# MDFahimAnjum/AliasFree-Diffusion-Models-PyTorch

Hardware: AMD Instinct MI355X
Metric: train_step_images_per_sec (higher is better)
Workload: dtype f32; 1 GPU; CIFAR-10 32x32x3 synthetic, UNet variant=3 (Config D), batch 256/GPU, T=1000, AdamW lr 3e-4, random-init weights (seed 42); global_batch=256, parallelism=dp1, hip_graph=True, launch_mode=lanes

## Files before the change

### aliasfree-diffusion-models-pytorch_amd/csrc/attn.hip

```cpp
#include "common.h"

namespace afd {

constexpr int kTile = 64;
constexpr int kChunk = 8;

using f2 = __attribute__((ext_vector_type(2))) float;
constexpr float kLog2e = 1.4426950408889634f, kLn2 = 0.6931471805599453f;

template <int D> struct RowVec {
  static __device__ __forceinline__ void load(const float* __restrict__ p, f2 (&v)[D / 2]) {
    if constexpr (D % 4 == 0) {
#pragma unroll
      for (int j = 0; j < D / 4; ++j) {
        const float4 t = reinterpret_cast<const float4*>(p)[j];
        v[2 * j] = (f2){t.x, t.y}; v[2 * j + 1] = (f2){t.z, t.w};
      }
    } else {
      const float2 t = *reinterpret_cast<const float2*>(p);
      v[0] = (f2){t.x, t.y};
    }
  }
};
template <int P> __device__ __forceinline__ float dot2(const f2 (&a)[P], const f2 (&b)[P]) {
  f2 t = a[0] * b[0];
#pragma unroll
  for (int i = 1; i < P; ++i) t = __builtin_elementwise_fma(a[i], b[i], t);
  return t.x + t.y;
}
template <int P> __device__ __forceinline__ void axpy2(f2 (&acc)[P], float s, const f2 (&v)[P]) {
  const f2 ss = {s, s};
#pragma unroll
  for (int i = 0; i < P; ++i) acc[i] = __builtin_elementwise_fma(ss, v[i], acc[i]);
}

template <int D, int NT>
__device__ __forceinline__ void stage_rows(const float* __restrict__ src, float* __restrict__ dst, int r0, int L, float mul) {
  constexpr int Q4 = D * kTile / 4;
  if constexpr (Q4 % NT == 0) {
    if ((L & 3) == 0) {
      constexpr int CAP = D >= 64 ? 2 : 8;
      constexpr int N4 = Q4 / NT, CH = N4 < CAP ? N4 : CAP;
#pragma unroll
      for (int e0 = 0; e0 < N4; e0 += CH) {
        float4 v[CH];
#pragma unroll
        for (int e = 0; e < CH; ++e) {
          const int i = threadIdx.x + NT * (e0 + e), j = i / (kTile / 4), rr = 4 * (i % (kTile / 4));
          v[e] = (r0 + rr < L) ? *reinterpret_cast<const float4*>(src + (long)j * L + r0 + rr) : make_float4(0.f, 0.f, 0.f, 0.f);
        }
#pragma unroll
        for (int e = 0; e < CH; ++e) {
          const int i = threadIdx.x + NT * (e0 + e), j = i / (kTile / 4), rr = 4 * (i % (kTile / 4));
          dst[rr * D + j] = v[e].x * mul; dst[(rr + 1) * D + j] = v[e].y * mul;
          dst[(rr + 2) * D + j] = v[e].z * mul; dst[(rr + 3) * D + j] = v[e].w * mul;
        }
      }
      return;
    }
  }
#pragma unroll 4
  for (int i = threadIdx.x; i < D * kTile; i += NT) {
    const int j = i / kTile, rr = i % kTile;
    dst[rr * D + j] = (r0 + rr < L) ? src[(long)j * L + r0 + rr] * mul : 0.f;
  }
}

template <int D, int R, int NT>
__global__ __launch_bounds__(NT) void attn_fwd_k(const float* __restrict__ qkv, float* __restrict__ o,
                                                  float* __restrict__ lse, int heads, int L, float scale) {
  constexpr int P = D / 2;
  __shared__ __attribute__((aligned(16))) float Ks[kTile * D];
  __shared__ __attribute__((aligned(16))) float Vs[kTile * D];
  const int b = blockIdx.z, h = blockIdx.y;
  const int C = heads * D;
  const int q0 = blockIdx.x * NT * R + threadIdx.x;
  const float* qp = qkv + ((long)b * 3 * C + h * D) * L;
  const float* kp = qp + (long)C * L;
  const float* vp = kp + (long)C * L;
  f2 q[R][P], acc[R][P];
  float m[R], l[R];
#pragma unroll
  for (int r = 0; r < R; ++r) {
    const int qi = q0 + r * NT;
    m[r] = -INFINITY; l[r] = 0.f;
#pragma unroll
    for (int j = 0; j < D; ++j) q[r][j >> 1][j & 1] = qi < L ? qp[(long)j * L + qi] * (scale * kLog2e) : 0.f;
#pragma unroll
    for (int i = 0; i < P; ++i) acc[r][i] = (f2){0.f, 0.f};
  }
  for (int k0 = 0; k0 < L; k0 += kTile) {
    __syncthreads();
    stage_rows<D, NT>(kp, Ks, k0, L, 1.f);
    stage_rows<D, NT>(vp, Vs, k0, L, 1.f);
    __syncthreads();
    const int nk = min(kTile, L - k0);
    for (int c0 = 0; c0 < nk; c0 += kChunk) {
      float s[R][kChunk], cm[R];
#pragma unroll
      for (int r = 0; r < R; ++r) cm[r] = m[r];
#pragma unroll
      for (int u = 0; u < kChunk; ++u) {
        f2 kv[P];
        RowVec<D>::load(Ks + (c0 + u) * D, kv);
        const bool in = c0 + u < nk;
#pragma unroll
        for (int r = 0; r < R; ++r) {
          s[r][u] = in ? dot2<P>(q[r], kv) : -INFINITY;
          cm[r] = fmaxf(cm[r], s[r][u]);
        }
      }
#pragma unroll
      for (int r = 0; r < R; ++r) {
        const float alpha = __builtin_amdgcn_exp2f(m[r] - cm[r]);
        l[r] *= alpha;
#pragma unroll
        for (int i = 0; i < P; ++i) acc[r][i] *= alpha;
        m[r] = cm[r];
      }
#pragma unroll
      for (int u = 0; u < kChunk; ++u) {
        f2 vv[P];
        RowVec<D>::load(Vs + (c0 + u) * D, vv);
#pragma unroll
        for (int r = 0; r < R; ++r) {
          const float p = __builtin_amdgcn_exp2f(s[r][u] - cm[r]);
          l[r] += p;
          axpy2<P>(acc[r], p, vv);
        }
      }
    }
  }
#pragma unroll
  for (int r = 0; r < R; ++r) {
    const int qi = q0 + r * NT;
    if (qi < L) {
      const float inv = 1.0f / l[r];
      float* op = o + ((long)b * C + h * D) * L + qi;
#pragma unroll
      for (int j = 0; j < D; ++j) op[(long)j * L] = acc[r][j >> 1][j & 1] * inv;
      lse[((long)b * heads + h) * L + qi] = (m[r] + __builtin_amdgcn_logf(l[r])) * kLn2;
    }
  }
}

template <int D, int R, int NT>
__global__ __launch_bounds__(NT) void attn_bwd_dq_k(const float* __restrict__ qkv, const float* __restrict__ o,
                                                     const float* __restrict__ d_o, const float* __restrict__ lse,
                                                     float* __restrict__ dqkv, float* __restrict__ delta_out,
                                                     int heads, int L, float scale) {
  constexpr int P = D / 2;
  __shared__ __attribute__((aligned(16))) float Ks[kTile * D];
  __shared__ __attribute__((aligned(16))) float Vs[kTile * D];
  const int b = blockIdx.z, h = blockIdx.y;
  const int C = heads * D;
  const int q0 = blockIdx.x * NT * R + threadIdx.x;
  const float* qp = qkv + ((long)b * 3 * C + h * D) * L;
  const float* kp = qp + (long)C * L;
  const float* vp = kp + (long)C * L;
  const long obase = ((long)b * C + h * D) * L;
  f2 q[R][P], go[R][P], dq[R][P];
  float delta[R], ls[R];
#pragma unroll
  for (int r = 0; r < R; ++r) {
    const int qi = q0 + r * NT;
    const bool live = qi < L;
    delta[r] = 0.f;
#pragma unroll
    for (int j = 0; j < D; ++j) {
      const float g = live ? d_o[obase + (long)j * L + qi] : 0.f;
      q[r][j >> 1][j & 1] = live ? qp[(long)j * L + qi] * (scale * kLog2e) : 0.f;
      go[r][j >> 1][j & 1] = g;
      delta[r] += g * (live ? o[obase + (long)j * L + qi] : 0.f);
    }
#pragma unroll
    for (int i = 0; i < P; ++i) dq[r][i] = (f2){0.f, 0.f};
    ls[r] = live ? lse[((long)b * heads + h) * L + qi] * kLog2e : 0.f;
    if (live) delta_out[((long)b * heads + h) * L + qi] = delta[r];
  }
  for (int k0 = 0; k0 < L; k0 += kTile) {
    __syncthreads();
    stage_rows<D, NT>(kp, Ks, k0, L, 1.f);
    stage_rows<D, NT>(vp, Vs, k0, L, 1.f);
    __syncthreads();
    const int nk = min(kTile, L - k0);
#pragma unroll 2
    for (int u = 0; u < nk; ++u) {
      f2 kv[P], vv[P];
      RowVec<D>::load(Ks + u * D, kv);
      RowVec<D>::load(Vs + u * D, vv);
#pragma unroll
      for (int r = 0; r < R; ++r) {
        const float sc = dot2<P>(q[r], kv), dp = dot2<P>(go[r], vv);
        const float ds = __builtin_amdgcn_exp2f(sc - ls[r]) * (dp - delta[r]);
        axpy2<P>(dq[r], ds, kv);
      }
    }
  }
#pragma unroll
  for (int r = 0; r < R; ++r) {
    const int qi = q0 + r * NT;
    if (qi < L) {
      float* dqp = dqkv + ((long)b * 3 * C + h * D) * L + qi;
#pragma unroll
      for (int j = 0; j < D; ++j) dqp[(long)j * L] = dq[r][j >> 1][j & 1] * scale;
    }
  }
}

template <int D, int R, int NT>
__global__ __launch_bounds__(NT) void attn_bwd_dkv_k(const float* __restrict__ qkv, const float* __restrict__ d_o,
                                                      const float* __restrict__ lse, const float* __restrict__ delta,
                                                      float* __restrict__ dqkv, int heads, int L, float scale) {
  constexpr int P = D / 2;
  __shared__ __attribute__((aligned(16))) float Qs[kTile * D];
  __shared__ __attribute__((aligned(16))) float Gs[kTile * D];
  __shared__ float Ls[kTile];
  __shared__ float Ds[kTile];
  const int b = blockIdx.z, h = blockIdx.y;
  const int C = heads * D;
  const int kq0 = blockIdx.x * NT * R + threadIdx.x;
  const float* qp = qkv + ((long)b * 3 * C + h * D) * L;
  const float* kp = qp + (long)C * L;
  const float* vp = kp + (long)C * L;
  const float* gp = d_o + ((long)b * C + h * D) * L;
  const float* lp = lse + ((long)b * heads + h) * L;
  const float* dlp = delta + ((long)b * heads + h) * L;
  f2 k[R][P], v[R][P], dk[R][P], dv[R][P];
#pragma unroll
  for (int r = 0; r < R; ++r) {
    const int ki = kq0 + r * NT;
#pragma unroll
    for (int j = 0; j < D; ++j) {
      k[r][j >> 1][j & 1] = ki < L ? kp[(long)j * L + ki] : 0.f;
      v[r][j >> 1][j & 1] = ki < L ? vp[(long)j * L + ki] : 0.f;
    }
#pragma unroll
    for (int i = 0; i < P; ++i) { dk[r][i] = (f2){0.f, 0.f}; dv[r][i] = (f2){0.f, 0.f}; }
  }
  for (int t0 = 0; t0 < L; t0 += kTile) {
    __syncthreads();
    stage_rows<D, NT>(qp, Qs, t0, L, scale * kLog2e);
    stage_rows<D, NT>(gp, Gs, t0, L, 1.f);
    for (int i = threadIdx.x; i < kTile; i += NT) {
      const bool in = t0 + i < L;
      Ls[i] = in ? lp[t0 + i] * kLog2e : INFINITY;
      Ds[i] = in ? dlp[t0 + i] : 0.f;
    }
    __syncthreads();
    const int nq = min(kTile, L - t0);
#pragma unroll 2
    for (int u = 0; u < nq; ++u) {
      f2 qv[P], gv[P];
      RowVec<D>::load(Qs + u * D, qv);
      RowVec<D>::load(Gs + u * D, gv);
      const float lsu = Ls[u], dlu = Ds[u];
#pragma unroll
      for (int r = 0; r < R; ++r) {
        const float sc = dot2<P>(qv, k[r]), dp = dot2<P>(gv, v[r]);
        const float p = __builtin_amdgcn_exp2f(sc - lsu);
        const float ds = p * (dp - dlu);
        axpy2<P>(dv[r], p, gv);
        axpy2<P>(dk[r], ds, qv);
      }
    }
  }
#pragma unroll
  for (int r = 0; r < R; ++r) {
    const int ki = kq0 + r * NT;
    if (ki < L) {
      float* dkp = dqkv + ((long)b * 3 * C + C + h * D) * L + ki;
      float* dvp = dkp + (long)C * L;
#pragma unroll
      for (int j = 0; j < D; ++j) { dkp[(long)j * L] = dk[r][j >> 1][j & 1] * kLn2; dvp[(long)j * L] = dv[r][j >> 1][j & 1]; }
    }
  }
}

}
using namespace afd;

template <int R> static inline void attn_geometry(int B, int heads, int L, dim3& grid, dim3& block) {
  const int rows = (L + R - 1) / R;
  block = dim3(rows <= 64 ? 64 : (rows <= 128 ? 128 : 256));
  grid = dim3((L + block.x * R - 1) / (block.x * R), heads, B);
}
template <int D, int R> static void launch_fwd(const float* qkv, float* o, float* lse, int B, int heads, int L, float sc, hipStream_t s) {
  dim3 grid, block; attn_geometry<R>(B, heads, L, grid, block);
  if (block.x == 64) hipLaunchKernelGGL((attn_fwd_k<D, R, 64>), grid, block, 0, s, qkv, o, lse, heads, L, sc);
  else if (block.x == 128) hipLaunchKernelGGL((attn_fwd_k<D, R, 128>), grid, block, 0, s, qkv, o, lse, heads, L, sc);
  else hipLaunchKernelGGL((attn_fwd_k<D, R, 256>), grid, block, 0, s, qkv, o, lse, heads, L, sc);
}
template <int D, int R> static void launch_dq(const float* qkv, const float* o, const float* d_o, const float* lse, float* dqkv,
                                              float* delta, int B, int heads, int L, float sc, hipStream_t s) {
  dim3 grid, block; attn_geometry<R>(B, heads, L, grid, block);
  if (block.x == 64) hipLaunchKernelGGL((attn_bwd_dq_k<D, R, 64>), grid, block, 0, s, qkv, o, d_o, lse, dqkv, delta, heads, L, sc);
  else if (block.x == 128) hipLaunchKernelGGL((attn_bwd_dq_k<D, R, 128>), grid, block, 0, s, qkv, o, d_o, lse, dqkv, delta, heads, L, sc);
  else hipLaunchKernelGGL((attn_bwd_dq_k<D, R, 256>), grid, block, 0, s, qkv, o, d_o, lse, dqkv, delta, heads, L, sc);
}
template <int D, int R> static void launch_dkv(const float* qkv, const float* d_o, const float* lse, const float* delta, float* dqkv,
                                               int B, int heads, int L, float sc, hipStream_t s) {
  dim3 grid, block; attn_geometry<R>(B, heads, L, grid, block);
  if (block.x == 64) hipLaunchKernelGGL((attn_bwd_dkv_k<D, R, 64>), grid, block, 0, s, qkv, d_o, lse, delta, dqkv, heads, L, sc);
  else if (block.x == 128) hipLaunchKernelGGL((attn_bwd_dkv_k<D, R, 128>), grid, block, 0, s, qkv, d_o, lse, delta, dqkv, heads, L, sc);
  else hipLaunchKernelGGL((attn_bwd_dkv_k<D, R, 256>), grid, block, 0, s, qkv, d_o, lse, delta, dqkv, heads, L, sc);
}

namespace afd {
bool attn_mfma8_ok(int d, int L);
void attn_pv_set(int m);
bool attn_fused_bwd(const float* qkv, const float* o, const float* d_o, const float* lse, float* dqkv, float* delta, int B, int heads,
                    int d, int L, float sc, hipStream_t s);
void attn_mfma8_fwd(const float* qkv, float* o, float* lse, int B, int heads, int d, int L, float sc, hipStream_t s);
void attn_mfma8_bwd_dq(const float* qkv, const float* o, const float* d_o, const float* lse, float* dqkv, float* delta,
                       int B, int heads, int d, int L, float sc, hipStream_t s);
void attn_mfma8_bwd_dkv(const float* qkv, const float* d_o, const float* lse, const float* delta, float* dqkv, int B, int heads, int L,
                        float sc, hipStream_t s);
}
static int g_attn_mfma_bwd_all = 1;
static int g_attn_rows = 0;

extern "C" {

int afd_debug_attn_rows(int r) {
  if (r == 20 || r == 21) { attn_pv_set(r - 20); return AFD_OK; }
  if (r == 10 || r == 11) { g_attn_mfma_bwd_all = r - 10; return AFD_OK; }
  AFD_REQUIRE(r == 0 || r == 1 || r == 2 || r == 4, "afd_debug_attn_rows: r must be 0, 1, 2, 4 (rows per lane of the VALU kernels), 10, 11, 20 or 21");
  g_attn_rows = r;
  return AFD_OK;
}

int afd_attn_fwd(const float* qkv, float* o, float* lse, int B, int heads, int d, int L, afd_stream_t st) {
  AFD_REQUIRE(qkv && o && lse && B > 0 && heads > 0 && L > 0, "afd_attn_fwd: bad argument");
  AFD_REQUIRE(d == 2 || d == 4 || d == 8 || d == 16 || d == 32 || d == 64, "afd_attn_fwd: head dim %d not in {2,4,8,16,32,64}", d);
  AFD_REQUIRE(B <= 65535 && heads <= 65535, "afd_attn_fwd: grid too large");
  hipStream_t s = as_stream(st);
  const float sc = 1.0f / sqrtf((float)d);
  if (g_attn_rows == 0 && attn_mfma8_ok(d, L)) { attn_mfma8_fwd(qkv, o, lse, B, heads, d, L, sc, s); return check_launch("afd_attn_fwd"); }
  switch (d) {
    case 2:  launch_fwd<2, 4>(qkv, o, lse, B, heads, L, sc, s); break;
    case 4:  launch_fwd<4, 4>(qkv, o, lse, B, heads, L, sc, s); break;
    case 8:
      if (g_attn_rows == 1 || (g_attn_rows == 0 && L < 1024)) launch_fwd<8, 1>(qkv, o, lse, B, heads, L, sc, s);
      else if (g_attn_rows == 4) launch_fwd<8, 4>(qkv, o, lse, B, heads, L, sc, s);
      else launch_fwd<8, 2>(qkv, o, lse, B, heads, L, sc, s);
      break;
    case 16: if (L <= 64) launch_fwd<16, 1>(qkv, o, lse, B, heads, L, sc, s); else launch_fwd<16, 2>(qkv, o, lse, B, heads, L, sc, s); break;
    case 32: if (L <= 64) launch_fwd<32, 1>(qkv, o, lse, B, heads, L, sc, s); else launch_fwd<32, 2>(qkv, o, lse, B, heads, L, sc, s); break;
    default: launch_fwd<64, 1>(qkv, o, lse, B, heads, L, sc, s); break;
  }
  return check_launch("afd_attn_fwd");
}

int afd_attn_bwd(const float* qkv, const float* o, const float* d_o, const float* lse, float* dqkv, float* delta_ws,
                 int B, int heads, int d, int L, afd_stream_t st) {
  AFD_REQUIRE(qkv && o && d_o && lse && dqkv && delta_ws && B > 0 && heads > 0 && L > 0, "afd_attn_bwd: bad argument");
  AFD_REQUIRE(d == 2 || d == 4 || d == 8 || d == 16 || d == 32 || d == 64, "afd_attn_bwd: head dim %d not in {2,4,8,16,32,64}", d);
  AFD_REQUIRE(B <= 65535 && heads <= 65535, "afd_attn_bwd: grid too large");
  hipStream_t s = as_stream(st);
  const float sc = 1.0f / sqrtf((float)d);
  if (g_attn_rows == 0 && attn_mfma8_ok(d, L) && (L < 1024 || g_attn_mfma_bwd_all)) {
    if (attn_fused_bwd(qkv, o, d_o, lse, dqkv, delta_ws, B, heads, d, L, sc, s)) return check_launch("afd_attn_bwd");
    attn_mfma8_bwd_dq(qkv, o, d_o, lse, dqkv, delta_ws, B, heads, d, L, sc, s);
    if (d == 8) attn_mfma8_bwd_dkv(qkv, d_o, lse, delta_ws, dqkv, B, heads, L, sc, s);
    else launch_dkv<16, 2>(qkv, d_o, lse, delta_ws, dqkv, B, heads, L, sc, s);
    return check_launch("afd_attn_bwd");
  }
  switch (d) {
    case 2:  launch_dq<2, 4>(qkv, o, d_o, lse, dqkv, delta_ws, B, heads, L, sc, s); break;
    case 4:  launch_dq<4, 4>(qkv, o, d_o, lse, dqkv, delta_ws, B, heads, L, sc, s); break;
    case 8:
      if (g_attn_rows == 1 || (g_attn_rows == 0 && L < 1024)) launch_dq<8, 1>(qkv, o, d_o, lse, dqkv, delta_ws, B, heads, L, sc, s);
      else if (g_attn_rows == 4) launch_dq<8, 4>(qkv, o, d_o, lse, dqkv, delta_ws, B, heads, L, sc, s);
      else launch_dq<8, 2>(qkv, o, d_o, lse, dqkv, delta_ws, B, heads, L, sc, s);
      break;
    case 16: if (L <= 64) launch_dq<16, 1>(qkv, o, d_o, lse, dqkv, delta_ws, B, heads, L, sc, s); else launch_dq<16, 2>(qkv, o, d_o, lse, dqkv, delta_ws, B, heads, L, sc, s); break;
    case 32: if (L <= 64) launch_dq<32, 1>(qkv, o, d_o, lse, dqkv, delta_ws, B, heads, L, sc, s); else launch_dq<32, 2>(qkv, o, d_o, lse, dqkv, delta_ws, B, heads, L, sc, s); break;
    default: launch_dq<64, 1>(qkv, o, d_o, lse, dqkv, delta_ws, B, heads, L, sc, s); break;
  }
  switch (d) {
    case 2:  launch_dkv<2, 4>(qkv, d_o, lse, delta_ws, dqkv, B, heads, L, sc, s); break;
    case 4:  launch_dkv<4, 4>(qkv, d_o, lse, delta_ws, dqkv, B, heads, L, sc, s); break;
    case 8:
      if (g_attn_rows == 1 || (g_attn_rows == 0 && L < 1024)) launch_dkv<8, 1>(qkv, d_o, lse, delta_ws, dqkv, B, heads, L, sc, s);
      else if (g_attn_rows == 4) launch_dkv<8, 4>(qkv, d_o, lse, delta_ws, dqkv, B, heads, L, sc, s);
      else launch_dkv<8, 2>(qkv, d_o, lse, delta_ws, dqkv, B, heads, L, sc, s);
      break;
    case 16: if (L <= 64) launch_dkv<16, 1>(qkv, d_o, lse, delta_ws, dqkv, B, heads, L, sc, s); else launch_dkv<16, 2>(qkv, d_o, lse, delta_ws, dqkv, B, heads, L, sc, s); break;
    case 32: launch_dkv<32, 1>(qkv, d_o, lse, delta_ws, dqkv, B, heads, L, sc, s); break;
    default: launch_dkv<64, 1>(qkv, d_o, lse, delta_ws, dqkv, B, heads, L, sc, s); break;
  }
  return check_launch("afd_attn_bwd");
}

}
```

Measured before the change: 38420 images/s.

## Add register-resident MFMA attention kernels for short sequences with head dim 16/32

Adds new forward and backward attention kernels for head dims 16/32 and sequence lengths up to 64, where one wavefront holds a whole (batch, head) pair in registers and computes QK^T and PV with 16x16x4 f32 MFMA. The backward pass recomputes softmax and splits into a dQ kernel and a dK/dV kernel, with no delta workspace pass. These replace the VALU tiled kernels for small attention layers at low-resolution UNet stages, aiming to cut scalar FLOP cost and launches. In exchange, the attention matrix is recomputed twice in backward and register pressure is high for T=4 with D=32.

```diff
diff --git a/aliasfree-diffusion-models-pytorch_amd/csrc/attn.hip b/aliasfree-diffusion-models-pytorch_amd/csrc/attn.hip
--- a/aliasfree-diffusion-models-pytorch_amd/csrc/attn.hip
+++ b/aliasfree-diffusion-models-pytorch_amd/csrc/attn.hip
@@ -317,15 +317,27 @@
 void attn_mfma8_bwd_dkv(const float* qkv, const float* d_o, const float* lse, const float* delta, float* dqkv, int B, int heads, int L,
                         float sc, hipStream_t s);
 }
+namespace afd {
+bool attn_small_ok(int d, int L);
+void attn_small_fwd_launch(const float* qkv, float* o, float* lse, int B, int heads, int d, int L, float sc, hipStream_t s);
+void attn_small_bwd_launch(const float* qkv, const float* d_o, float* dqkv, int B, int heads, int d, int L, float sc,
+                           hipStream_t s);
+}
 static int g_attn_mfma_bwd_all = 1;
 static int g_attn_rows = 0;
 
+static int g_attn_small = 1;
+static inline bool attn_small_use(int B, int heads, int d, int L) {
+  return g_attn_small && g_attn_rows == 0 && attn_small_ok(d, L) && (long)B * heads <= (1L << 30);
+}
+
 extern "C" {
 
 int afd_debug_attn_rows(int r) {
   if (r == 20 || r == 21) { attn_pv_set(r - 20); return AFD_OK; }
+  if (r == 30 || r == 31) { g_attn_small = r - 30; return AFD_OK; }
   if (r == 10 || r == 11) { g_attn_mfma_bwd_all = r - 10; return AFD_OK; }
-  AFD_REQUIRE(r == 0 || r == 1 || r == 2 || r == 4, "afd_debug_attn_rows: r must be 0, 1, 2, 4 (rows per lane of the VALU kernels), 10, 11, 20 or 21");
+  AFD_REQUIRE(r == 0 || r == 1 || r == 2 || r == 4, "afd_debug_attn_rows: r must be 0, 1, 2, 4 (rows per lane of the VALU kernels), 10, 11, 20, 21, 30 or 31");
   g_attn_rows = r;
   return AFD_OK;
 }
@@ -337,6 +349,10 @@
   hipStream_t s = as_stream(st);
   const float sc = 1.0f / sqrtf((float)d);
   if (g_attn_rows == 0 && attn_mfma8_ok(d, L)) { attn_mfma8_fwd(qkv, o, lse, B, heads, d, L, sc, s); return check_launch("afd_attn_fwd"); }
+  if (attn_small_use(B, heads, d, L) && aligned16(qkv)) {
+    attn_small_fwd_launch(qkv, o, lse, B, heads, d, L, sc, s);
+    return check_launch("afd_attn_fwd");
+  }
   switch (d) {
     case 2:  launch_fwd<2, 4>(qkv, o, lse, B, heads, L, sc, s); break;
     case 4:  launch_fwd<4, 4>(qkv, o, lse, B, heads, L, sc, s); break;
@@ -366,6 +382,10 @@
     else launch_dkv<16, 2>(qkv, d_o, lse, delta_ws, dqkv, B, heads, L, sc, s);
     return check_launch("afd_attn_bwd");
   }
+  if (attn_small_use(B, heads, d, L) && aligned16(qkv) && aligned16(d_o)) {
+    attn_small_bwd_launch(qkv, d_o, dqkv, B, heads, d, L, sc, s);
+    return check_launch("afd_attn_bwd");
+  }
   switch (d) {
     case 2:  launch_dq<2, 4>(qkv, o, d_o, lse, dqkv, delta_ws, B, heads, L, sc, s); break;
     case 4:  launch_dq<4, 4>(qkv, o, d_o, lse, dqkv, delta_ws, B, heads, L, sc, s); break;
diff --git a/aliasfree-diffusion-models-pytorch_amd/csrc/attn_small.hip b/aliasfree-diffusion-models-pytorch_amd/csrc/attn_small.hip
--- /dev/null
+++ b/aliasfree-diffusion-models-pytorch_amd/csrc/attn_small.hip
@@ -0,0 +1,256 @@
+#include "common.h"
+
+namespace afd {
+
+namespace {
+using f4 = __attribute__((ext_vector_type(4))) float;
+constexpr float kLog2e = 1.4426950408889634f, kLn2 = 0.6931471805599453f;
+
+__device__ __forceinline__ f4 mfma4(float a, float b, f4 c) { return __builtin_amdgcn_mfma_f32_16x16x4f32(a, b, c, 0, 0, 0); }
+
+__device__ __forceinline__ float col_max(float v) {
+  v = fmaxf(v, __shfl_xor(v, 16, kWave));
+  return fmaxf(v, __shfl_xor(v, 32, kWave));
+}
+__device__ __forceinline__ float col_sum(float v) {
+  v += __shfl_xor(v, 16, kWave);
+  return v + __shfl_xor(v, 32, kWave);
+}
+__device__ __forceinline__ float row_max(float v) {
+#pragma unroll
+  for (int o = 1; o < 16; o <<= 1) v = fmaxf(v, __shfl_xor(v, o, kWave));
+  return v;
+}
+__device__ __forceinline__ float row_sum(float v) {
+#pragma unroll
+  for (int o = 1; o < 16; o <<= 1) v += __shfl_xor(v, o, kWave);
+  return v;
+}
+
+template <int D, int T>
+__device__ __forceinline__ void load_free(const float* __restrict__ x, int c, int g, float mul, float (&r)[T][D / 4]) {
+#pragma unroll
+  for (int t = 0; t < T; ++t)
+#pragma unroll
+    for (int s = 0; s < D / 4; ++s) r[t][s] = x[(4 * s + g) * (16 * T) + 16 * t + c] * mul;
+}
+template <int D, int T>
+__device__ __forceinline__ void load_contr(const float* __restrict__ x, int c, int g, f4 (&r)[D / 16][T]) {
+#pragma unroll
+  for (int jt = 0; jt < D / 16; ++jt)
+#pragma unroll
+    for (int t = 0; t < T; ++t) r[jt][t] = *reinterpret_cast<const f4*>(x + (16 * jt + c) * (16 * T) + 16 * t + 4 * g);
+}
+template <int D, int T>
+__device__ __forceinline__ void prod_feat(const float (&a)[T][D / 4], const float (&b)[T][D / 4], f4 (&acc)[T][T]) {
+#pragma unroll
+  for (int s = 0; s < D / 4; ++s)
+#pragma unroll
+    for (int i = 0; i < T; ++i)
+#pragma unroll
+      for (int j = 0; j < T; ++j) acc[i][j] = mfma4(a[i][s], b[j][s], acc[i][j]);
+}
+template <int D, int T>
+__device__ __forceinline__ void prod_tok(const f4 (&x)[D / 16][T], const f4 (&acc)[T][T], f4 (&out)[D / 16][T]) {
+#pragma unroll
+  for (int m = 0; m < T; ++m)
+#pragma unroll
+    for (int r = 0; r < 4; ++r)
+#pragma unroll
+      for (int jt = 0; jt < D / 16; ++jt)
+#pragma unroll
+        for (int n = 0; n < T; ++n) out[jt][n] = mfma4(x[jt][m][r], acc[m][n][r], out[jt][n]);
+}
+template <int D, int T>
+__device__ __forceinline__ void store_t(float* __restrict__ dst, int c, int g, const f4 (&out)[D / 16][T], const float (&mul)[T]) {
+#pragma unroll
+  for (int jt = 0; jt < D / 16; ++jt)
+#pragma unroll
+    for (int n = 0; n < T; ++n)
+#pragma unroll
+      for (int r = 0; r < 4; ++r) dst[(16 * jt + 4 * g + r) * (16 * T) + 16 * n + c] = out[jt][n][r] * mul[n];
+}
+template <int A, int B> __device__ __forceinline__ void zero(f4 (&x)[A][B]) {
+#pragma unroll
+  for (int i = 0; i < A; ++i)
+#pragma unroll
+    for (int j = 0; j < B; ++j) x[i][j] = (f4){0.f, 0.f, 0.f, 0.f};
+}
+}
+
+template <int D, int T>
+__global__ __launch_bounds__(256) void attn_small_fwd(const float* __restrict__ qkv, float* __restrict__ o, float* __restrict__ lse,
+                                                       int pairs, int heads, float scale) {
+  constexpr int L = 16 * T;
+  const int pair = blockIdx.x * 4 + __builtin_amdgcn_readfirstlane(threadIdx.x >> 6);
+  if (pair >= pairs) return;
+  const int c = threadIdx.x & 15, g = (threadIdx.x & 63) >> 4;
+  const int b = pair / heads, h = pair - b * heads, C = heads * D;
+  const float* qp = qkv + ((long)b * 3 * C + h * D) * L;
+  const float* kp = qp + (long)C * L;
+  const float* vp = kp + (long)C * L;
+  float qa[T][D / 4], ka[T][D / 4];
+  f4 vt[D / 16][T];
+  load_free<D, T>(kp, c, g, 1.f, ka);
+  load_free<D, T>(qp, c, g, scale * kLog2e, qa);
+  load_contr<D, T>(vp, c, g, vt);
+  f4 st[T][T];
+  zero(st);
+  prod_feat<D, T>(ka, qa, st);
+  float one[T];
+#pragma unroll
+  for (int qt = 0; qt < T; ++qt) {
+    float m = st[0][qt][0];
+#pragma unroll
+    for (int kt = 0; kt < T; ++kt)
+#pragma unroll
+      for (int r = 0; r < 4; ++r) m = fmaxf(m, st[kt][qt][r]);
+    m = col_max(m);
+    float l = 0.f;
+#pragma unroll
+    for (int kt = 0; kt < T; ++kt)
+#pragma unroll
+      for (int r = 0; r < 4; ++r) { st[kt][qt][r] = __builtin_amdgcn_exp2f(st[kt][qt][r] - m); l += st[kt][qt][r]; }
+    l = col_sum(l);
+    const float inv = 1.0f / l;
+#pragma unroll
+    for (int kt = 0; kt < T; ++kt)
+#pragma unroll
+      for (int r = 0; r < 4; ++r) st[kt][qt][r] *= inv;
+    one[qt] = 1.f;
+    if (g == 0) lse[(long)pair * L + 16 * qt + c] = (m + __builtin_amdgcn_logf(l)) * kLn2;
+  }
+  f4 ot[D / 16][T];
+  zero(ot);
+  prod_tok<D, T>(vt, st, ot);
+  store_t<D, T>(o + ((long)b * C + h * D) * L, c, g, ot, one);
+}
+
+template <int D, int T, int PART>
+__global__ __launch_bounds__(256) void attn_small_bwd(const float* __restrict__ qkv, const float* __restrict__ d_o,
+                                                       float* __restrict__ dqkv, int pairs, int heads, float scale) {
+  constexpr int L = 16 * T;
+  const int pair = blockIdx.x * 4 + __builtin_amdgcn_readfirstlane(threadIdx.x >> 6);
+  if (pair >= pairs) return;
+  const int c = threadIdx.x & 15, g = (threadIdx.x & 63) >> 4;
+  const int b = pair / heads, h = pair - b * heads, C = heads * D;
+  const float* qp = qkv + ((long)b * 3 * C + h * D) * L;
+  const float* kp = qp + (long)C * L;
+  const float* vp = kp + (long)C * L;
+  const float* gp = d_o + ((long)b * C + h * D) * L;
+  float* dqp = dqkv + ((long)b * 3 * C + h * D) * L;
+  float qa[T][D / 4], ka[T][D / 4], va[T][D / 4], ga[T][D / 4];
+  load_free<D, T>(kp, c, g, 1.f, ka);
+  load_free<D, T>(qp, c, g, scale * kLog2e, qa);
+  load_free<D, T>(vp, c, g, 1.f, va);
+  load_free<D, T>(gp, c, g, 1.f, ga);
+  float sc[T], one[T];
+#pragma unroll
+  for (int t = 0; t < T; ++t) { sc[t] = scale; one[t] = 1.f; }
+  if constexpr (PART == 0) {
+    f4 st[T][T], dp[T][T];
+    zero(st); zero(dp);
+    prod_feat<D, T>(ka, qa, st);
+    prod_feat<D, T>(va, ga, dp);
+#pragma unroll
+    for (int qt = 0; qt < T; ++qt) {
+      float m = st[0][qt][0], l = 0.f, dl = 0.f;
+#pragma unroll
+      for (int kt = 0; kt < T; ++kt)
+#pragma unroll
+        for (int r = 0; r < 4; ++r) m = fmaxf(m, st[kt][qt][r]);
+      m = col_max(m);
+#pragma unroll
+      for (int kt = 0; kt < T; ++kt)
+#pragma unroll
+        for (int r = 0; r < 4; ++r) { st[kt][qt][r] = __builtin_amdgcn_exp2f(st[kt][qt][r] - m); l += st[kt][qt][r]; }
+      l = col_sum(l);
+      const float inv = 1.0f / l;
+#pragma unroll
+      for (int kt = 0; kt < T; ++kt)
+#pragma unroll
+        for (int r = 0; r < 4; ++r) { st[kt][qt][r] *= inv; dl = fmaf(st[kt][qt][r], dp[kt][qt][r], dl); }
+      dl = col_sum(dl);
+#pragma unroll
+      for (int kt = 0; kt < T; ++kt)
+#pragma unroll
+        for (int r = 0; r < 4; ++r) st[kt][qt][r] *= dp[kt][qt][r] - dl;
+    }
+    f4 kt4[D / 16][T], dq[D / 16][T];
+    load_contr<D, T>(kp, c, g, kt4);
+    zero(dq);
+    prod_tok<D, T>(kt4, st, dq);
+    store_t<D, T>(dqp, c, g, dq, sc);
+  } else {
+    f4 s2[T][T], dp[T][T];
+    zero(s2); zero(dp);
+    prod_feat<D, T>(qa, ka, s2);
+    prod_feat<D, T>(ga, va, dp);
+    f4 ds[T][T];
+#pragma unroll
+    for (int qt = 0; qt < T; ++qt) {
+#pragma unroll
+      for (int r = 0; r < 4; ++r) {
+        float m = s2[qt][0][r], l = 0.f, dl = 0.f;
+#pragma unroll
+        for (int kt = 1; kt < T; ++kt) m = fmaxf(m, s2[qt][kt][r]);
+        m = row_max(m);
+#pragma unroll
+        for (int kt = 0; kt < T; ++kt) { s2[qt][kt][r] = __builtin_amdgcn_exp2f(s2[qt][kt][r] - m); l += s2[qt][kt][r]; }
+        const float inv = 1.0f / row_sum(l);
+#pragma unroll
+        for (int kt = 0; kt < T; ++kt) { s2[qt][kt][r] *= inv; dl = fmaf(s2[qt][kt][r], dp[qt][kt][r], dl); }
+        dl = row_sum(dl);
+#pragma unroll
+        for (int kt = 0; kt < T; ++kt) ds[qt][kt][r] = s2[qt][kt][r] * (dp[qt][kt][r] - dl);
+      }
+    }
+    f4 x4[D / 16][T], out[D / 16][T];
+    load_contr<D, T>(gp, c, g, x4);
+    zero(out);
+    prod_tok<D, T>(x4, s2, out);
+    store_t<D, T>(dqp + 2 * (long)C * L, c, g, out, one);
+    load_contr<D, T>(qp, c, g, x4);
+    zero(out);
+    prod_tok<D, T>(x4, ds, out);
+    store_t<D, T>(dqp + (long)C * L, c, g, out, sc);
+  }
+}
+
+bool attn_small_ok(int d, int L) { return (d == 16 || d == 32) && L % 16 == 0 && L >= 16 && L <= 64; }
+
+template <int D> static void small_fwd_d(const float* qkv, float* o, float* lse, int pairs, int heads, int T, float sc, hipStream_t s) {
+  const dim3 grid((pairs + 3) / 4), block(256);
+  switch (T) {
+    case 1: hipLaunchKernelGGL((attn_small_fwd<D, 1>), grid, block, 0, s, qkv, o, lse, pairs, heads, sc); break;
+    case 2: hipLaunchKernelGGL((attn_small_fwd<D, 2>), grid, block, 0, s, qkv, o, lse, pairs, heads, sc); break;
+    case 3: hipLaunchKernelGGL((attn_small_fwd<D, 3>), grid, block, 0, s, qkv, o, lse, pairs, heads, sc); break;
+    default: hipLaunchKernelGGL((attn_small_fwd<D, 4>), grid, block, 0, s, qkv, o, lse, pairs, heads, sc); break;
+  }
+}
+template <int D> static void small_bwd_d(const float* qkv, const float* d_o, float* dqkv, int pairs, int heads, int T,
+                                         float sc, hipStream_t s) {
+  const dim3 grid((pairs + 3) / 4), block(256);
+  switch (T) {
+    case 1: hipLaunchKernelGGL((attn_small_bwd<D, 1, 0>), grid, block, 0, s, qkv, d_o, dqkv, pairs, heads, sc);
+            hipLaunchKernelGGL((attn_small_bwd<D, 1, 1>), grid, block, 0, s, qkv, d_o, dqkv, pairs, heads, sc); break;
+    case 2: hipLaunchKernelGGL((attn_small_bwd<D, 2, 0>), grid, block, 0, s, qkv, d_o, dqkv, pairs, heads, sc);
+            hipLaunchKernelGGL((attn_small_bwd<D, 2, 1>), grid, block, 0, s, qkv, d_o, dqkv, pairs, heads, sc); break;
+    case 3: hipLaunchKernelGGL((attn_small_bwd<D, 3, 0>), grid, block, 0, s, qkv, d_o, dqkv, pairs, heads, sc);
+            hipLaunchKernelGGL((attn_small_bwd<D, 3, 1>), grid, block, 0, s, qkv, d_o, dqkv, pairs, heads, sc); break;
+    default: hipLaunchKernelGGL((attn_small_bwd<D, 4, 0>), grid, block, 0, s, qkv, d_o, dqkv, pairs, heads, sc);
+             hipLaunchKernelGGL((attn_small_bwd<D, 4, 1>), grid, block, 0, s, qkv, d_o, dqkv, pairs, heads, sc); break;
+  }
+}
+
+void attn_small_fwd_launch(const float* qkv, float* o, float* lse, int B, int heads, int d, int L, float sc, hipStream_t s) {
+  if (d == 16) small_fwd_d<16>(qkv, o, lse, B * heads, heads, L / 16, sc, s);
+  else small_fwd_d<32>(qkv, o, lse, B * heads, heads, L / 16, sc, s);
+}
+void attn_small_bwd_launch(const float* qkv, const float* d_o, float* dqkv, int B, int heads, int d, int L, float sc,
+                           hipStream_t s) {
+  if (d == 16) small_bwd_d<16>(qkv, d_o, dqkv, B * heads, heads, L / 16, sc, s);
+  else small_bwd_d<32>(qkv, d_o, dqkv, B * heads, heads, L / 16, sc, s);
+}
+
+}
```

Result: faster. 39040 images/s (median of 6 runs) (+1.6%).
